# pymoc/pymoc

Measured on AMD Instinct MI355X. Metric: column-timesteps/sec (ensemble) at nz=100, higher is better.
Workload: dtype f64; 1 GPU; BASELINE configs[1]: 1024 independent Columns x nz=100 fp64 per GPU, static wA, do_conv on odd members, dt=30 d (pymoc_amd.configs.config2); columns_per_gpu=1024, nz=100, kernel=k_column_steps<64,2,6,true,true>, parallelism=ensemble sharded over 1 GPU(s), RCCL gather (root) of the final state

## Files before the change

### pymoc_amd/csrc/column.hip.h

```cpp
#pragma once
#include <type_traits>
#include "common.hip.h"

namespace pm {

template <int P>
struct ColGrid {
  double z[P];
  double dz[P];
  double dzc[P];
  double rdz[P], rdzc[P];
  double rdz_l[P], rdzc_l[P];
};
template <int P>
struct ColRegs {
  double b[P];
  double kap[P];
  double area[P];
  double dAk[P];
  double rarea[P];
  double rarea_l[P];
  double area_u, rarea_u, rarea_lu;
};

template <int P>
__device__ __forceinline__ void load_levels(double (&out)[P], const double *__restrict__ row,
                                            int lg, int nz, int lvl0 = 0) {
  if constexpr (P == 2) {
    if (lvl0 == 0 && (nz & 1) == 0 && (((unsigned long long)row) & 15ull) == 0ull) {
      const int i0 = lg * 2 < nz - 2 ? lg * 2 : nz - 2;
      const double2 v = *reinterpret_cast<const double2 *>(row + i0);
      out[0] = v.x;
      out[1] = v.y;
      return;
    }
  }
#pragma unroll
  for (int p = 0; p < P; ++p) {
    const int i = lvl0 + lg * P + p;
    out[p] = row[i < nz ? i : nz - 1];
  }
}

template <int P>
__device__ __forceinline__ double level_value(const double (&x)[P], int j) {
  const int jl = __builtin_amdgcn_readfirstlane(j / P);
  const int jp = __builtin_amdgcn_readfirstlane(j % P);
  double out = 0.;
#pragma unroll
  for (int p = 0; p < P; ++p) {
    const int lo = __builtin_amdgcn_readlane(__double2loint(x[p]), jl);
    const int hi = __builtin_amdgcn_readlane(__double2hiint(x[p]), jl);
    const double v = __hiloint2double(hi, lo);
    out = (p == 0 || jp == p) ? v : out;
  }
  return out;
}

__device__ __forceinline__ double lane_value(double x, int lane) {
  const int lo = __builtin_amdgcn_readlane(__double2loint(x), lane);
  const int hi = __builtin_amdgcn_readlane(__double2hiint(x), lane);
  return __hiloint2double(hi, lo);
}

template <int P>
struct ConvCache {
  unsigned long long mask[P];
  double zconv;
  bool valid = false;
};

template <int G, int P>
__device__ __forceinline__ bool col_convect(double (&b)[P], const double (&z)[P],
                                            double bs, double N2min, int lg, int lane,
                                            int nz, const double *__restrict__ zg,
                                            ConvCache<P> *cache = nullptr) {
  const unsigned long long gm = group_mask<G>(lane);
  bool ind[P];
  unsigned long long im[P];
  unsigned long long anym = 0ull;
#pragma unroll
  for (int p = 0; p < P; ++p) {
    const int i = lg * P + p;
    ind[p] = (i < nz) && (b[p] > bs);
    im[p] = __builtin_amdgcn_ballot_w64(ind[p]);
    anym |= im[p] & gm;
  }
  if (__builtin_expect(anym != 0ull, 0)) {
    double zconv;
    bool hit = false;
    if constexpr (G == 64) {
      if (cache != nullptr && cache->valid) {
        hit = true;
#pragma unroll
        for (int p = 0; p < P; ++p) hit = hit && (cache->mask[p] == im[p]);
      }
    }
    if (hit) {
      zconv = cache->zconv;
    } else {
      int jmax = 0;
#pragma unroll
      for (int p = 0; p < P; ++p) {
        const int i = lg * P + p;
        const unsigned long long m = __builtin_amdgcn_ballot_w64((i < nz) && !ind[p]) & gm;
        if (m != 0ull) {
          const int hl = 63 - __clzll((long long)m);
          const int j = (hl % G) * P + p;
          jmax = j > jmax ? j : jmax;
        }
      }
      if constexpr (G == 64) {
        zconv = level_value<P>(z, jmax);
        if (cache != nullptr) {
#pragma unroll
          for (int p = 0; p < P; ++p) cache->mask[p] = im[p];
          cache->zconv = zconv;
          cache->valid = true;
        }
      } else {
        zconv = zg[jmax];
      }
    }
#pragma unroll
    for (int p = 0; p < P; ++p) {
      const double adj = bs + N2min * (z[p] - zconv);
      b[p] = ind[p] ? adj : b[p];
    }
    return true;
  }
#pragma unroll
  for (int p = 0; p < P; ++p)
    if (lg * P + p == nz - 1) b[p] = bs;
  return false;
}

template <int P>
__device__ __forceinline__ void col_convect_cached(double (&b)[P], const double (&z)[P],
                                                   double bs, double N2min, int lane, int nz,
                                                   ConvCache<P> &cc) {
  bool ind[P];
  unsigned long long im[P], anym = 0ull;
  bool same = cc.valid;
#pragma unroll
  for (int p = 0; p < P; ++p) {
    ind[p] = (lane * P + p < nz) && (b[p] > bs);
    im[p] = __builtin_amdgcn_ballot_w64(ind[p]);
    anym |= im[p];
    same = same && (im[p] == cc.mask[p]);
  }
  if (__builtin_expect(!same, 0)) {
    int jmax = 0;
#pragma unroll
    for (int p = 0; p < P; ++p) {
      const unsigned long long m = __builtin_amdgcn_ballot_w64((lane * P + p < nz) && !ind[p]);
      if (m != 0ull) {
        const int j = (63 - __clzll((long long)m)) * P + p;
        jmax = j > jmax ? j : jmax;
      }
    }
    cc.zconv = level_value<P>(z, jmax);
#pragma unroll
    for (int p = 0; p < P; ++p) cc.mask[p] = im[p];
    cc.valid = true;
  }
  const bool none = anym == 0ull;
#pragma unroll
  for (int p = 0; p < P; ++p) {
    const double adj = bs + N2min * (z[p] - cc.zconv);
    b[p] = ind[p] ? adj : b[p];
    if (lane * P + p == nz - 1) b[p] = none ? bs : b[p];
  }
}

template <int G, int P, int DIV, bool BC = true, bool WEFF = false, bool UA = false,
          bool FLUXFMA = (DIV == 2 || DIV >= 6)>
__device__ __forceinline__ void col_vertadvdiff(const ColGrid<P> &g, ColRegs<P> &r,
                                                const double (&wA)[P],
                                                double dt, bool do_conv, double bs,
                                                double bbot, bool use_bzbot,
                                                double bzbot, int lg, int nz,
                                                int lvl0 = 0) {
  if (BC && !do_conv) {
#pragma unroll
    for (int p = 0; p < P; ++p)
      if (lvl0 + lg * P + p == nz - 1) r.b[p] = bs;
  }
  const double nb0 = from_next_lane_z(r.b[0]);
  double bup[P];
#pragma unroll
  for (int p = 0; p < P; ++p) bup[p] = (p < P - 1) ? r.b[p + 1 < P ? p + 1 : p] : nb0;
  if (BC && lvl0 + lg * P == 0) r.b[0] = use_bzbot ? (bup[0] - bzbot * g.dz[0]) : bbot;

  if constexpr (DIV == 4) {
    double d_up[P];
#pragma unroll
    for (int p = 0; p < P; ++p) d_up[p] = bup[p] - r.b[p];
    const double pd = from_prev_lane_z(d_up[P - 1]);
#pragma unroll
    for (int p = 0; p < P; ++p) {
      const double d_dn = (p > 0) ? d_up[p > 0 ? p - 1 : 0] : pd;
      r.b[p] = __builtin_fma(r.kap[p], d_up[p], __builtin_fma(r.dAk[p], d_dn, r.b[p]));
    }
    return;
  }
  double bz[P];
  {
    double num[P], q[P], rr[P];
#pragma unroll
    for (int p = 0; p < P; ++p) num[p] = bup[p] - r.b[p];
    if constexpr (DIV == 2) {
#pragma unroll
      for (int p = 0; p < P; ++p) rr[p] = num[p] * g.rdz_l[p];
#pragma unroll
      for (int p = 0; p < P; ++p) q[p] = __builtin_fma(num[p], g.rdz[p], rr[p]);
#pragma unroll
      for (int p = 0; p < P; ++p) rr[p] = __builtin_fma(-g.dz[p], q[p], num[p]);
#pragma unroll
      for (int p = 0; p < P; ++p) q[p] = __builtin_fma(rr[p], g.rdz[p], q[p]);
    } else if constexpr (DIV == 7 || DIV == 8) {
#pragma unroll
      for (int p = 0; p < P; ++p) rr[p] = num[p] * g.rdz_l[p];
#pragma unroll
      for (int p = 0; p < P; ++p) q[p] = __builtin_fma(num[p], g.rdz[p], rr[p]);
    } else if constexpr (DIV == 6) {
#pragma unroll
      for (int p = 0; p < P; ++p) q[p] = num[p] * g.rdz[p];
#pragma unroll
      for (int p = 0; p < P; ++p) rr[p] = __builtin_fma(-g.dz[p], q[p], num[p]);
#pragma unroll
      for (int p = 0; p < P; ++p) q[p] = __builtin_fma(rr[p], g.rdz[p], q[p]);
    } else if constexpr (DIV == 1 || DIV == 3 || DIV == 5) {
#pragma unroll
      for (int p = 0; p < P; ++p) q[p] = num[p] * g.rdz[p];
#pragma unroll
      for (int p = 0; p < P; ++p) rr[p] = __builtin_fma(-g.dz[p], q[p], num[p]);
#pragma unroll
      for (int p = 0; p < P; ++p) q[p] = __builtin_fma(rr[p], g.rdz[p], q[p]);
#pragma unroll
      for (int p = 0; p < P; ++p) rr[p] = __builtin_fma(-g.dz[p], q[p], num[p]);
#pragma unroll
      for (int p = 0; p < P; ++p) q[p] = __builtin_fma(rr[p], g.rdz[p], q[p]);
    } else {
#pragma unroll
      for (int p = 0; p < P; ++p) q[p] = num[p] / g.dz[p];
    }
    if constexpr (DIV != 0) {
#pragma unroll
      for (int p = 0; p < P; ++p) bz[p] = q[p];
    } else {
#pragma unroll
      for (int p = 0; p < P; ++p) bz[p] = (lvl0 + lg * P + p < nz - 1) ? q[p] : 0.0;
    }
  }
  const double pbz = from_prev_lane_z(bz[P - 1]);
  double bz_dn[P], dbz[P], flx[P], bzz[P], adv[P];
#pragma unroll
  for (int p = 0; p < P; ++p) {
    bz_dn[p] = (p > 0) ? bz[p > 0 ? p - 1 : 0] : pbz;
    dbz[p] = bz[p] - bz_dn[p];
    const double weff = WEFF ? wA[p] : wA[p] - r.dAk[p];
    if constexpr (FLUXFMA) {
      const double wn = (weff < 0.0) ? -weff : 0.0, wp = (weff < 0.0) ? 0.0 : -weff;
      flx[p] = __builtin_fma(wn, bz[p], wp * bz_dn[p]);
    } else {
      const double bzu = (weff < 0.0) ? bz[p] : bz_dn[p];
      flx[p] = (-weff) * bzu;
    }
  }
  if constexpr (DIV == 2) {
    double r1[P], r2[P];
#pragma unroll
    for (int p = 0; p < P; ++p) {
      r1[p] = dbz[p] * g.rdzc_l[p];
      r2[p] = flx[p] * (UA ? r.rarea_lu : r.rarea_l[p]);
    }
#pragma unroll
    for (int p = 0; p < P; ++p) {
      bzz[p] = __builtin_fma(dbz[p], g.rdzc[p], r1[p]);
      adv[p] = __builtin_fma(flx[p], (UA ? r.rarea_u : r.rarea[p]), r2[p]);
    }
#pragma unroll
    for (int p = 0; p < P; ++p) {
      r1[p] = __builtin_fma(-g.dzc[p], bzz[p], dbz[p]);
      r2[p] = __builtin_fma(-(UA ? r.area_u : r.area[p]), adv[p], flx[p]);
    }
#pragma unroll
    for (int p = 0; p < P; ++p) {
      bzz[p] = __builtin_fma(r1[p], g.rdzc[p], bzz[p]);
      adv[p] = __builtin_fma(r2[p], (UA ? r.rarea_u : r.rarea[p]), adv[p]);
    }
  } else if constexpr (DIV == 6) {
    double r1[P], r2[P];
#pragma unroll
    for (int p = 0; p < P; ++p) {
      bzz[p] = dbz[p] * g.rdzc[p];
      adv[p] = flx[p] * (UA ? r.rarea_u : r.rarea[p]);
    }
#pragma unroll
    for (int p = 0; p < P; ++p) {
      r1[p] = __builtin_fma(-g.dzc[p], bzz[p], dbz[p]);
      r2[p] = __builtin_fma(-(UA ? r.area_u : r.area[p]), adv[p], flx[p]);
    }
#pragma unroll
    for (int p = 0; p < P; ++p) {
      bzz[p] = __builtin_fma(r1[p], g.rdzc[p], bzz[p]);
      adv[p] = __builtin_fma(r2[p], (UA ? r.rarea_u : r.rarea[p]), adv[p]);
    }
  } else if constexpr (DIV == 8) {
    double r1[P], r2[P];
#pragma unroll
    for (int p = 0; p < P; ++p) {
      r1[p] = dbz[p] * g.rdzc_l[p];
      r2[p] = flx[p] * (UA ? r.rarea_lu : r.rarea_l[p]);
    }
#pragma unroll
    for (int p = 0; p < P; ++p) {
      bzz[p] = __builtin_fma(dbz[p], g.rdzc[p], r1[p]);
      adv[p] = __builtin_fma(flx[p], (UA ? r.rarea_u : r.rarea[p]), r2[p]);
    }
  } else if constexpr (DIV == 7) {
    double r1[P], r2[P];
#pragma unroll
    for (int p = 0; p < P; ++p) {
      r1[p] = dbz[p] * g.rdzc_l[p];
      adv[p] = flx[p] * (UA ? r.rarea_u : r.rarea[p]);
    }
#pragma unroll
    for (int p = 0; p < P; ++p) {
      bzz[p] = __builtin_fma(dbz[p], g.rdzc[p], r1[p]);
      r2[p] = __builtin_fma(-(UA ? r.area_u : r.area[p]), adv[p], flx[p]);
    }
#pragma unroll
    for (int p = 0; p < P; ++p) adv[p] = __builtin_fma(r2[p], (UA ? r.rarea_u : r.rarea[p]), adv[p]);
  } else if constexpr (DIV == 5) {
    double r1[P];
#pragma unroll
    for (int p = 0; p < P; ++p) {
      bzz[p] = dbz[p] * g.rdzc[p];
      adv[p] = div_by_recip2(flx[p], r.area_u, r.rarea_u, r.rarea_lu);
    }
#pragma unroll
    for (int k = 0; k < 2; ++k) {
#pragma unroll
      for (int p = 0; p < P; ++p) r1[p] = __builtin_fma(-g.dzc[p], bzz[p], dbz[p]);
#pragma unroll
      for (int p = 0; p < P; ++p) bzz[p] = __builtin_fma(r1[p], g.rdzc[p], bzz[p]);
    }
  } else if constexpr (DIV == 3) {
    double r1[P];
#pragma unroll
    for (int p = 0; p < P; ++p) {
      bzz[p] = dbz[p] * g.rdzc[p];
      adv[p] = flx[p] / (UA ? r.area_u : r.area[p]);
    }
#pragma unroll
    for (int k = 0; k < 2; ++k) {
#pragma unroll
      for (int p = 0; p < P; ++p) r1[p] = __builtin_fma(-g.dzc[p], bzz[p], dbz[p]);
#pragma unroll
      for (int p = 0; p < P; ++p) bzz[p] = __builtin_fma(r1[p], g.rdzc[p], bzz[p]);
    }
  } else if constexpr (DIV == 1) {
    double r1[P], r2[P];
#pragma unroll
    for (int p = 0; p < P; ++p) {
      bzz[p] = dbz[p] * g.rdzc[p];
      adv[p] = flx[p] * (UA ? r.rarea_u : r.rarea[p]);
    }
#pragma unroll
    for (int k = 0; k < 2; ++k) {
#pragma unroll
      for (int p = 0; p < P; ++p) {
        r1[p] = __builtin_fma(-g.dzc[p], bzz[p], dbz[p]);
        r2[p] = __builtin_fma(-(UA ? r.area_u : r.area[p]), adv[p], flx[p]);
      }
#pragma unroll
      for (int p = 0; p < P; ++p) {
        bzz[p] = __builtin_fma(r1[p], g.rdzc[p], bzz[p]);
        adv[p] = __builtin_fma(r2[p], (UA ? r.rarea_u : r.rarea[p]), adv[p]);
      }
    }
  } else {
#pragma unroll
    for (int p = 0; p < P; ++p) {
      bzz[p] = dbz[p] / g.dzc[p];
      adv[p] = flx[p] / (UA ? r.area_u : r.area[p]);
    }
  }
#pragma unroll
  for (int p = 0; p < P; ++p) {
    const int i = lvl0 + lg * P + p;
    const bool interior = (i >= 1) && (i <= nz - 2);
    const double db_dt = adv[p] + r.kap[p] * bzz[p];
    if constexpr (DIV == 0) {
      const double nb = r.b[p] + dt * db_dt;
      r.b[p] = interior ? nb : r.b[p];
    } else {
      r.b[p] = r.b[p] + (interior ? dt : 0.0) * db_dt;
    }
  }
}

template <int P>
__device__ __forceinline__ void col_horadv(ColRegs<P> &r, const double (&vdx)[P],
                                           const double (&bin)[P], double dt, int lg,
                                           int nz) {
#pragma unroll
  for (int p = 0; p < P; ++p) {
    const int i = lg * P + p;
    if (i < nz && vdx[p] > 0.0) {
      const double db = bin[p] - r.b[p];
      r.b[p] = r.b[p] + dt * vdx[p] * db / r.area[p];
    }
  }
}

template <int P>
__device__ __forceinline__ bool col_inputs_in_fast_range(const ColGrid<P> &g, const ColRegs<P> &r,
                                                         const double (&wA)[P], double dt,
                                                         double bs, double bbot, double bzbot,
                                                         double N2min, int lg, int nz) {
  bool ok = in_fast_div_range(dt) && in_fast_div_range(bs) && in_fast_div_range(bbot) &&
            in_fast_div_range(bzbot) && in_fast_div_range(N2min);
#pragma unroll
  for (int p = 0; p < P; ++p) {
    const bool top = lg * P + p >= nz - 1;
    ok = ok && in_fast_div_range(r.b[p]) && in_fast_div_range(wA[p]) &&
         in_fast_div_range(r.dAk[p]) && in_fast_div_range(wA[p] - r.dAk[p]) &&
         in_fast_div_range(r.kap[p]) && in_fast_div_range(r.area[p]) && r.area[p] != 0.0 &&
         in_fast_div_range(g.z[p]) && (top || (in_fast_div_range(g.dz[p]) && g.dz[p] != 0.0)) &&
         in_fast_div_range(g.dzc[p]) && g.dzc[p] != 0.0;
  }
  return ok;
}

template <int P>
__device__ __forceinline__ bool col_state_in_fast_range(const ColRegs<P> &r, const double (&wA)[P]) {
  int ok = 1;
#pragma unroll
  for (int p = 0; p < P; ++p)
    ok &= (int)in_fast_div_range(r.b[p]) & (int)in_fast_div_range(wA[p] - r.dAk[p]);
  return ok != 0;
}

template <int P, int DIV = 1>
__device__ __forceinline__ void col_load_grid(ColGrid<P> &g, const pm_columns &c, int lg,
                                              int lvl0 = 0) {
  const int nz = c.nz;
#pragma unroll
  for (int p = 0; p < P; ++p) {
    const int i = lvl0 + lg * P + p;
    const int ic = i < nz ? i : nz - 1;
    const int iu = ic + 1 < nz ? ic + 1 : nz - 1;
    const int id = ic > 0 ? ic - 1 : 0;
    const double zc = c.z[ic];
    g.z[p] = zc;
    g.dz[p] = c.z[iu] - zc;
    g.dzc[p] = 0.5 * (g.dz[p] + (zc - c.z[id]));
    if constexpr (DIV != 0 && DIV != 4) {
      g.rdz[p] = (i < nz - 1) ? 1.0 / g.dz[p] : 0.0;
      g.rdzc[p] = 1.0 / g.dzc[p];
    } else {
      g.rdz[p] = g.rdzc[p] = 0.0;
    }
    if constexpr (DIV == 2) {
      g.rdz_l[p] = (i < nz - 1) ? recip_lo(g.dz[p], g.rdz[p]) : 0.0;
      g.rdzc_l[p] = recip_lo(g.dzc[p], g.rdzc[p]);
    } else {
      g.rdz_l[p] = g.rdzc_l[p] = 0.0;
    }
  }
}

template <int P, int DIV = 1>
__device__ __forceinline__ void col_load_static(ColRegs<P> &r, const pm_columns &c,
                                                int col, int sel, int lg, int lvl0 = 0,
                                                bool uniform_area = false, bool weff_in = false) {
  const int nz = c.nz;
  const size_t base = (size_t)col * nz;
  const size_t sbase = ((size_t)sel * c.ncols + col) * nz;
  load_levels<P>(r.kap, c.kappa + sbase, lg, nz, lvl0);
  if (!weff_in) {
    load_levels<P>(r.dAk, c.dAkappa + sbase, lg, nz, lvl0);
  } else {
#pragma unroll
    for (int p = 0; p < P; ++p) r.dAk[p] = 0.0;
  }
  if (uniform_area) {
    const double a0 = c.area[base];
    const double ra = (DIV != 0 && DIV != 4) ? 1.0 / a0 : 0.0;
    const double ral = DIV == 2 ? recip_lo(a0, ra) : 0.0;
#pragma unroll
    for (int p = 0; p < P; ++p) {
      r.area[p] = a0;
      r.rarea[p] = ra;
      r.rarea_l[p] = ral;
    }
    return;
  }
  load_levels<P>(r.area, c.area + base, lg, nz, lvl0);
#pragma unroll
  for (int p = 0; p < P; ++p) {
    r.rarea[p] = (DIV != 0 && DIV != 4) ? 1.0 / r.area[p] : 0.0;
    r.rarea_l[p] = DIV == 2 ? recip_lo(r.area[p], r.rarea[p]) : 0.0;
  }
}

template <int P>
__device__ __forceinline__ void col_make_contracted(const ColGrid<P> &g, ColRegs<P> &r,
                                                    const double (&wA)[P], double dt, int lane,
                                                    int nz) {
  const double dz_prev_lane = from_prev_lane_z(g.dz[P - 1]);
#pragma unroll
  for (int p = 0; p < P; ++p) {
    const int i = lane * P + p;
    const bool interior = i >= 1 && i <= nz - 2;
    const double weff = wA[p] - r.dAk[p];
    const double dz_up = interior ? g.dz[p] : 1.0;
    const double dz_dn = interior ? ((p > 0) ? g.dz[p > 0 ? p - 1 : 0] : dz_prev_lane) : 1.0;
    const double dzc = interior ? g.dzc[p] : 1.0, area = interior ? r.area[p] : 1.0;
    const double wn = (weff < 0.0) ? -weff : 0.0, wp = (weff < 0.0) ? 0.0 : -weff;
    const double cu = dt * (r.kap[p] / (dzc * dz_up) + wn / (area * dz_up));
    const double cl = dt * (-r.kap[p] / (dzc * dz_dn) + wp / (area * dz_dn));
    r.kap[p] = interior ? cu : 0.0;
    r.dAk[p] = interior ? cl : 0.0;
  }
}

template <int P>
__device__ __forceinline__ unsigned conv_variant(const ConvCache<P> &cc) {
  unsigned need = 0u;
#pragma unroll
  for (int p = 0; p < P; ++p) need |= (cc.mask[p] != 0ull) ? (1u << p) : 0u;
  if constexpr (P <= 2) {
    return need;
  } else {
    return need ? (1u << P) - 1u : 0u;
  }
}

template <int P, int DIV, unsigned SEL, bool UA = false>
__device__ __forceinline__ int conv_spec_run(const ColGrid<P> &g, ColRegs<P> &r,
                                             const double (&wA)[P], double dt, double bs,
                                             double bbot, double N2min, int lane, int nz,
                                             ConvCache<P> &cc, int s, int nsteps) {
  constexpr int UNR = P <= 2 ? 16 : (P <= 4 ? 2 : 1);
  double adjv[P];
  double bs_eff[P];
  auto set_adj = [&]() {
#pragma unroll
    for (int p = 0; p < P; ++p)
      adjv[p] = (lane * P + p == 0) ? bbot : bs + N2min * (g.z[p] - cc.zconv);
  };
  set_adj();
#pragma unroll
  for (int p = 0; p < P; ++p) bs_eff[p] = (lane * P + p < nz) ? bs : __builtin_inf();
  double b_blk[P];
  unsigned long long acc;
  double bmax[P];
  auto spec = [&]() {
    unsigned long long im[P];
    bool ind[P];
#pragma unroll
    for (int p = 0; p < P; ++p) {
      if (((SEL >> p) & 1u) != 0u) {
        ind[p] = r.b[p] > bs_eff[p];
        im[p] = __builtin_amdgcn_ballot_w64(ind[p]);
      } else {
        bmax[p] = __builtin_fmax(bmax[p], r.b[p]);
      }
    }
#pragma unroll
    for (int p = 0; p < P; ++p) {
      if (((SEL >> p) & 1u) != 0u) r.b[p] = ind[p] ? adjv[p] : r.b[p];
    }
    col_vertadvdiff<64, P, DIV, false, false, UA>(g, r, wA, dt, true, bs, bbot, false, 0., lane, nz);
#pragma unroll
    for (int p = 0; p < P; ++p) {
      if (((SEL >> p) & 1u) != 0u) {
        unsigned long long x;
        asm("s_xor_b64 %0, %1, %2" : "=s"(x) : "s"(im[p]), "s"(cc.mask[p]) : "scc");
        acc |= x;
      }
    }
  };
  auto block_begin = [&]() {
    acc = 0ull;
#pragma unroll
    for (int p = 0; p < P; ++p) {
      b_blk[p] = r.b[p];
      bmax[p] = -__builtin_inf();
    }
  };
  auto block_bad = [&]() -> bool {
    bool conv = false;
#pragma unroll
    for (int p = 0; p < P; ++p)
      if (((SEL >> p) & 1u) == 0u) conv = conv || (bmax[p] > bs_eff[p]);
    if constexpr (SEL != (1u << P) - 1u) {
      unsigned long long any = __builtin_amdgcn_ballot_w64(conv);
      asm("" : "+s"(any));
      acc |= any;
    }
    return acc != 0ull;
  };
  auto redo = [&](int nb) {
#pragma unroll
    for (int p = 0; p < P; ++p) r.b[p] = b_blk[p];
    for (int k = 0; k < nb; ++k) {
      col_convect_cached<P>(r.b, g.z, bs, N2min, lane, nz, cc);
      if (lane == 0) r.b[0] = bbot;
      col_vertadvdiff<64, P, DIV, false, false, UA>(g, r, wA, dt, true, bs, bbot, false, 0., lane, nz);
    }
  };
  int pos = s, ret = -1;
  auto tier = [&](auto U) {
    constexpr int N = decltype(U)::value;
    int left = (nsteps - pos) / N;
    const int s_end = pos + left * N;
    for (; left > 0; --left) {
      block_begin();
#pragma unroll
      for (int k = 0; k < N; ++k) spec();
      if (__builtin_expect(block_bad(), 0)) {
        redo(N);
        if (conv_variant<P>(cc) != SEL) {
          ret = s_end - (left - 1) * N;
          left = 1;
        } else {
          set_adj();
        }
      }
    }
    pos = s_end;
  };
  if (UNR <= 4 || nsteps - pos >= 4 * UNR) tier(std::integral_constant<int, UNR>{});
  if (ret >= 0) return ret;
  if constexpr (UNR > 4) {
    tier(std::integral_constant<int, 4>{});
    if (ret >= 0) return ret;
  }
  if constexpr (UNR > 1) tier(std::integral_constant<int, 1>{});
  return ret >= 0 ? ret : nsteps;
}

template <int G, int P>
__device__ __forceinline__ void col_store_result(const pm_columns &c, const ColRegs<P> &r,
                                                 size_t base, int col, bool col_ok, int lg,
                                                 int lane, int nz) {
  bool bad = false;
  bool stored = false;
  if constexpr (P == 2) {
    if ((nz & 1) == 0 && (((unsigned long long)(c.b + base)) & 15ull) == 0ull) {
      if (lg * 2 < nz) {
        if (col_ok) *reinterpret_cast<double2 *>(c.b + base + lg * 2) = make_double2(r.b[0], r.b[1]);
        bad = !isfinite(r.b[0]) || !isfinite(r.b[1]);
      }
      stored = true;
    }
  }
  if (!stored) {
#pragma unroll
    for (int p = 0; p < P; ++p) {
      const int i = lg * P + p;
      if (i < nz) {
        if (col_ok) c.b[base + i] = r.b[p];
        bad |= !isfinite(r.b[p]);
      }
    }
  }
  if (c.nonfinite) {
    const unsigned long long m = __ballot(bad) & group_mask<G>(lane);
    if (lg == 0 && col_ok) c.nonfinite[col] = (m != 0ull) ? 1 : 0;
  }
}

template <int P>
__device__ __forceinline__ void col_pin(double (&b)[P]) {
#pragma unroll
  for (int p = 0; p < P; ++p) asm volatile("" : "+v"(b[p]));
}

template <int G, int P, int FAST, bool PLAIN, bool UA = false>
__global__ __launch_bounds__(256) void k_column_steps(
    pm_columns c, const double *__restrict__ wA_g, const double *__restrict__ vdx_g,
    const double *__restrict__ bin_g, double dt, int nsteps, int ops) {
  const int lane = threadIdx.x & (WAVE - 1);
  const int lg = threadIdx.x % G;
  int col_raw = (int)((blockIdx.x * (unsigned)blockDim.x + threadIdx.x) / G);
  constexpr bool FORMS = FAST == 6 && G == 64 && P <= 2 && PLAIN;
  if constexpr (FORMS) col_raw = __builtin_amdgcn_readfirstlane(col_raw);
  const bool col_ok = col_raw < c.ncols;
  const int col = col_ok ? col_raw : c.ncols - 1;
  const int nz = c.nz;
  const size_t base = (size_t)col * nz;

  ColGrid<P> g;
  ColRegs<P> r;
  const int sel = c.ksel ? c.ksel[col] : 0;
  const int flags = c.flags ? c.flags[col] : 0;
  col_load_grid<P, FAST>(g, c, lg);
  const bool ua = G == 64 && __builtin_amdgcn_readfirstlane(flags & PM_COL_UNIFORM_AREA) != 0;
  col_load_static<P, FAST>(r, c, col, sel, lg, 0, ua, (ops & PM_OP_WEFF) != 0);
  if constexpr (UA) {
    r.area_u = lane_value(r.area[0], 0);
    r.rarea_u = lane_value(r.rarea[0], 0);
    r.rarea_lu = lane_value(r.rarea_l[0], 0);
  }

  double wA[P], vdx[P], bin[P];
  load_levels<P>(r.b, c.b + base, lg, nz);
#pragma unroll
  for (int p = 0; p < P; ++p) wA[p] = vdx[p] = bin[p] = 0.0;
  const bool wA_row = !(PLAIN && (ops & PM_OP_WA_TWOBASIN) != 0 && col >= 2 * (c.ncols / 3));
  if (wA_g && wA_row) load_levels<P>(wA, wA_g + base, lg, nz);
  if constexpr (PLAIN) {
    if (ops & PM_OP_WA_PSI) {
      const int half = c.ncols >> 1;
      if (col < half) {
        if (bin_g) {
          double pso[P];
          load_levels<P>(pso, bin_g + base, lg, nz);
#pragma unroll
          for (int p = 0; p < P; ++p) wA[p] = (wA[p] - pso[p]) * 1e6;
        } else {
#pragma unroll
          for (int p = 0; p < P; ++p) wA[p] = wA[p] * 1e6;
        }
      } else {
#pragma unroll
        for (int p = 0; p < P; ++p) wA[p] = (-wA[p]) * 1e6;
      }
    }
  }
  if constexpr (PLAIN) {
    if (ops & PM_OP_WA_TWOBASIN) {
      const int third = c.ncols / 3;
      if (col < third) {
        double zon[P], pso[P];
        load_levels<P>(zon, vdx_g + base, lg, nz);
        load_levels<P>(pso, bin_g + base, lg, nz);
#pragma unroll
        for (int p = 0; p < P; ++p) wA[p] = (wA[p] + zon[p] - pso[p]) * 1e6;
      } else if (col < 2 * third) {
#pragma unroll
        for (int p = 0; p < P; ++p) wA[p] = (-wA[p]) * 1e6;
      } else {
        const size_t bp = (size_t)(col - third) * nz;
        double zon[P], pso[P];
        load_levels<P>(zon, vdx_g + bp, lg, nz);
        load_levels<P>(pso, bin_g + bp, lg, nz);
#pragma unroll
        for (int p = 0; p < P; ++p) wA[p] = (-zon[p] - pso[p]) * 1e6;
      }
    }
  }
  const bool wa_formed = (ops & (PM_OP_WA_PSI | PM_OP_WA_TWOBASIN)) != 0;
  if (vdx_g && !wa_formed) load_levels<P>(vdx, vdx_g + base, lg, nz);
  if (bin_g && !wa_formed) load_levels<P>(bin, bin_g + base, lg, nz);
  const bool do_conv = (flags & PM_COL_DO_CONV) != 0;
  const bool use_bzbot = (flags & PM_COL_BZBOT) != 0 && c.bzbot != nullptr;
  const double bs = c.bs[col];
  const double bbot = c.bbot[col];
  const double bzbot = use_bzbot ? c.bzbot[col] : 0.0;
  const double N2min = c.N2min[col];

  if constexpr (FAST != 0) {
    const bool vouched = G == 64 &&
                         __builtin_amdgcn_readfirstlane(flags & PM_COL_STATIC_IN_RANGE) != 0 &&
                         in_fast_div_range(dt);
    bool fast_ok;
    if (vouched)
      fast_ok = col_state_in_fast_range<P>(r, wA);
    else
      fast_ok = col_inputs_in_fast_range<P>(g, r, wA, dt, bs, bbot, bzbot, N2min, lg, nz);
    if (__builtin_expect(__ballot(!fast_ok) != 0ull, 0)) {
      for (int s = 0; s < nsteps; ++s) {
        if ((ops & PM_OP_CONVECT) && do_conv)
          col_convect<G, P>(r.b, g.z, bs, N2min, lg, lane, nz, c.z);
        col_pin<P>(r.b);
        if (ops & PM_OP_VERTADVDIFF)
          col_vertadvdiff<G, P, 0>(g, r, wA, dt, do_conv, bs, bbot, use_bzbot, bzbot, lg, nz);
        if ((ops & PM_OP_HORADV) && vdx_g) col_horadv<P>(r, vdx, bin, dt, lg, nz);
      }
      col_store_result<G, P>(c, r, base, col, col_ok, lg, lane, nz);
      return;
    }
  }

  if constexpr (FAST == 4) col_make_contracted<P>(g, r, wA, dt, lane, nz);

  auto plain_run = [&](auto DIVC) {
    constexpr int DIV = decltype(DIVC)::value;
    if (do_conv && use_bzbot) {
      for (int s = 0; s < nsteps; ++s) {
        col_convect<G, P>(r.b, g.z, bs, N2min, lg, lane, nz, c.z);
        col_vertadvdiff<G, P, DIV, true, false, UA>(g, r, wA, dt, true, bs, bbot, true, bzbot, lg, nz);
      }
    } else if (do_conv) {
      ConvCache<P> cc;
#pragma unroll
      for (int p = 0; p < P; ++p) cc.mask[p] = 0ull;
      cc.zconv = 0.;
      if constexpr (G == 64) {
        col_convect_cached<P>(r.b, g.z, bs, N2min, lane, nz, cc);
        if (lg == 0) r.b[0] = bbot;
        col_vertadvdiff<G, P, DIV, false, false, UA>(g, r, wA, dt, true, bs, bbot, false, 0., lg, nz);
        int s = 1;
        while (s < nsteps) {
          const unsigned v = conv_variant<P>(cc);
          if constexpr (P <= 2) {
            switch (v) {
              case 0: s = conv_spec_run<P, DIV, 0u, UA>(g, r, wA, dt, bs, bbot, N2min, lane, nz, cc, s, nsteps); break;
              case 1: s = conv_spec_run<P, DIV, 1u, UA>(g, r, wA, dt, bs, bbot, N2min, lane, nz, cc, s, nsteps); break;
              case 2: s = conv_spec_run<P, DIV, 2u, UA>(g, r, wA, dt, bs, bbot, N2min, lane, nz, cc, s, nsteps); break;
              default: s = conv_spec_run<P, DIV, 3u, UA>(g, r, wA, dt, bs, bbot, N2min, lane, nz, cc, s, nsteps); break;
            }
          } else {
            if (v == 0u)
              s = conv_spec_run<P, DIV, 0u, UA>(g, r, wA, dt, bs, bbot, N2min, lane, nz, cc, s, nsteps);
            else
              s = conv_spec_run<P, DIV, (1u << P) - 1u, UA>(g, r, wA, dt, bs, bbot, N2min, lane, nz, cc, s, nsteps);
          }
        }
      } else {
        for (int s = 0; s < nsteps; ++s) {
          col_convect<G, P>(r.b, g.z, bs, N2min, lg, lane, nz, c.z);
          if (lg == 0) r.b[0] = bbot;
          col_vertadvdiff<G, P, DIV, false, false, UA>(g, r, wA, dt, true, bs, bbot, false, 0., lg, nz);
        }
      }
    } else if (use_bzbot) {
      for (int s = 0; s < nsteps; ++s)
        col_vertadvdiff<G, P, DIV, true, false, UA>(g, r, wA, dt, false, bs, bbot, true, bzbot, lg, nz);
    } else {
#pragma unroll
      for (int p = 0; p < P; ++p) {
        if (lg * P + p == nz - 1) r.b[p] = bs;
        if (lg * P + p == 0) r.b[p] = bbot;
      }
      int s = 0;
      if constexpr (P <= 2) {
        for (; s + 4 <= nsteps; s += 4) {
          col_vertadvdiff<G, P, DIV, false, false, UA>(g, r, wA, dt, false, bs, bbot, false, 0., lg, nz);
          col_vertadvdiff<G, P, DIV, false, false, UA>(g, r, wA, dt, false, bs, bbot, false, 0., lg, nz);
          col_vertadvdiff<G, P, DIV, false, false, UA>(g, r, wA, dt, false, bs, bbot, false, 0., lg, nz);
          col_vertadvdiff<G, P, DIV, false, false, UA>(g, r, wA, dt, false, bs, bbot, false, 0., lg, nz);
        }
      }
      for (; s < nsteps; ++s)
        col_vertadvdiff<G, P, DIV, false, false, UA>(g, r, wA, dt, false, bs, bbot, false, 0., lg, nz);
    }
  };
  if constexpr (PLAIN) {
    if constexpr (FORMS) {
      const bool d2g = (c.reserved & PM_COLS_DIV3_PROVEN) != 0 && (c.reserved & PM_COLS_DIV2_GRID) != 0;
      if (d2g) {
#pragma unroll
        for (int p = 0; p < P; ++p) {
          const bool below_top = lg * P + p < nz - 1;
          g.rdz_l[p] = below_top ? recip_lo_div(g.dz[p], g.rdz[p]) : 0.0;
          g.rdzc_l[p] = below_top ? recip_lo_div(g.dzc[p], g.rdzc[p]) : 0.0;
        }
        if (__builtin_amdgcn_readfirstlane(flags & PM_COL_DIV2_AREA) != 0) {
          if constexpr (UA) {
            r.rarea_lu = lane_value(recip_lo_div(r.area_u, r.rarea_u), 0);
          } else {
#pragma unroll
            for (int p = 0; p < P; ++p) r.rarea_l[p] = recip_lo_div(r.area[p], r.rarea[p]);
          }
          plain_run(std::integral_constant<int, 8>{});
        } else {
          plain_run(std::integral_constant<int, 7>{});
        }
      } else {
        plain_run(std::integral_constant<int, 6>{});
      }
    } else {
      plain_run(std::integral_constant<int, FAST>{});
    }
  } else {
    for (int s = 0; s < nsteps; ++s) {
      if ((ops & PM_OP_CONVECT) && do_conv)
        col_convect<G, P>(r.b, g.z, bs, N2min, lg, lane, nz, c.z);
      col_pin<P>(r.b);
      if (ops & PM_OP_VERTADVDIFF)
        col_vertadvdiff<G, P, FAST, true, false, UA>(g, r, wA, dt, do_conv, bs, bbot, use_bzbot, bzbot, lg, nz);
      if ((ops & PM_OP_HORADV) && vdx_g) col_horadv<P>(r, vdx, bin, dt, lg, nz);
    }
  }

  col_store_result<G, P>(c, r, base, col, col_ok, lg, lane, nz);
}

template <int P>
struct ColStage {
  double b[P], wA[P], kap[P], area[P], dAk[P];
};
template <int P>
struct ColStageLean {
  double b[P], wA[P];
};

struct StreamScalars {
  int flags, sel;
  double bs, bbot, bzbot, N2min, area0, kbase;
  double ra, ral;
  __device__ __forceinline__ void load(const pm_columns &c, int col0, int cend, int lane) {
    const int col = col0 + lane < cend ? col0 + lane : cend - 1;
    flags = c.flags ? c.flags[col] : 0;
    sel = c.ksel ? c.ksel[col] : 0;
    bs = c.bs[col];
    bbot = c.bbot[col];
    N2min = c.N2min[col];
    bzbot = ((flags & PM_COL_BZBOT) != 0 && c.bzbot != nullptr) ? c.bzbot[col] : 0.0;
    area0 = (flags & PM_COL_UNIFORM_AREA) ? c.area[(size_t)col * c.nz] : 0.0;
    kbase = c.kappa_base ? c.kappa_base[col] : 0.0;
    ra = 1.0 / area0;
    ral = recip_lo(area0, ra);
  }
};

template <int P, bool AFF = false>
__device__ __forceinline__ void col_stage_load(ColStage<P> &s, const pm_columns &c,
                                               const double *__restrict__ wA_g, int col,
                                               int lane, bool weff_in, int flags, int sel,
                                               double area0) {
  const int nz = c.nz;
  const size_t base = (size_t)col * nz;
  const size_t sbase = ((size_t)sel * c.ncols + col) * nz;
  load_levels<P>(s.b, c.b + base, lane, nz);
  load_levels<P>(s.wA, wA_g + base, lane, nz);
  if constexpr (!AFF) load_levels<P>(s.kap, c.kappa + sbase, lane, nz);
  if ((flags & PM_COL_UNIFORM_AREA) == 0) {
    load_levels<P>(s.area, c.area + base, lane, nz);
  } else {
#pragma unroll
    for (int p = 0; p < P; ++p) s.area[p] = area0;
  }
  if (!weff_in) {
    load_levels<P>(s.dAk, c.dAkappa + sbase, lane, nz);
  } else {
#pragma unroll
    for (int p = 0; p < P; ++p) s.dAk[p] = 0.0;
  }
}

template <int P, int D, bool AFF = false, bool LEAN = false, bool VEC = false, bool D3 = false,
          int CPWU = 0, int WEFFT = -1, int UABT = -1>
__global__ __launch_bounds__(256) __attribute__((amdgpu_waves_per_eu((LEAN && P <= 2 && D <= 5) ? 4 : 1)))
void k_column_stream(pm_columns c,
                                                       const double *__restrict__ wA_g,
                                                       double dt, int nsteps, int cpw, bool dt_ok,
                                                       bool weff_in) {
  const int lane = threadIdx.x & (WAVE - 1);
  const int wave = (int)((blockIdx.x * (unsigned)blockDim.x + threadIdx.x) >> 6);
  const int col0 = __builtin_amdgcn_readfirstlane(wave * cpw);
  const int nz = c.nz;
  if (col0 >= c.ncols) return;
  const int cend = col0 + cpw < c.ncols ? col0 + cpw : c.ncols;

  StreamScalars sc;
  sc.load(c, col0, cend, lane);
  static_assert(!LEAN || AFF, "the lean ring needs the affine kappa");
  static_assert(!VEC || (LEAN && P == 2), "16-byte accesses: the lean form with two levels per lane");
  const int off2 = lane * 2 < nz - 2 ? lane * 2 : nz - 2;
  using Stage = typename std::conditional<LEAN, ColStageLean<P>, ColStage<P>>::type;
  auto flags_of = [&](int k) { return __builtin_amdgcn_readlane(sc.flags, k); };
  auto issue = [&](Stage &st, int col) {
    const int k = col - col0;
    if constexpr (VEC) {
      const size_t base = (size_t)col * nz;
      const double2 vb = *reinterpret_cast<const double2 *>(c.b + base + off2);
      const double2 vw = *reinterpret_cast<const double2 *>(wA_g + base + off2);
      st.b[0] = vb.x;
      st.b[P - 1] = vb.y;
      st.wA[0] = vw.x;
      st.wA[P - 1] = vw.y;
    } else if constexpr (LEAN) {
      const size_t base = (size_t)col * nz;
      load_levels<P>(st.b, c.b + base, lane, nz);
      load_levels<P>(st.wA, wA_g + base, lane, nz);
    } else if constexpr (CPWU > 0 && WEFFT >= 0 && UABT >= 0) {
      const int sel = __builtin_amdgcn_readlane(sc.sel, k);
      const size_t base = (size_t)col * nz, sbase = ((size_t)sel * c.ncols + col) * nz;
      load_levels<P>(st.b, c.b + base, lane, nz);
      load_levels<P>(st.wA, wA_g + base, lane, nz);
      if constexpr (!AFF) load_levels<P>(st.kap, c.kappa + sbase, lane, nz);
      if constexpr (UABT == 0) load_levels<P>(st.area, c.area + base, lane, nz);
      if constexpr (WEFFT == 0) load_levels<P>(st.dAk, c.dAkappa + sbase, lane, nz);
    } else {
      col_stage_load<P, AFF>(st, c, wA_g, col, lane, weff_in, flags_of(k),
                             __builtin_amdgcn_readlane(sc.sel, k), lane_value(sc.area0, k));
    }
  };
  ColGrid<P> g;
  col_load_grid<P, 1>(g, c, lane);
  double kprof[P];
#pragma unroll
  for (int p = 0; p < P; ++p) kprof[p] = 0.0;
  if constexpr (AFF) load_levels<P>(kprof, c.kappa_profile, lane, nz);
  Stage ring[D];
#pragma unroll
  for (int d = 0; d < D; ++d)
    if (col0 + d < cend) issue(ring[d], col0 + d);
  unsigned nf_bits = 0u;
  auto one_column = [&](int col, int d, bool prefetch, int kk) {
      ColRegs<P> r;
      double wA[P];
#pragma unroll
      for (int p = 0; p < P; ++p) {
        r.b[p] = ring[d].b[p];
        wA[p] = ring[d].wA[p];
        if constexpr (AFF)
          r.kap[p] = lane_value(sc.kbase, col - col0) + kprof[p];
        else
          r.kap[p] = ring[d].kap[p];
        if constexpr (LEAN) {
          r.area[p] = lane_value(sc.area0, col - col0);
          r.area_u = r.area[p];
          r.rarea_u = lane_value(sc.ra, col - col0);
          r.rarea_lu = lane_value(sc.ral, col - col0);
          r.dAk[p] = 0.0;
        } else if constexpr (CPWU > 0 && WEFFT >= 0 && UABT >= 0) {
          if constexpr (UABT == 1)
            r.area[p] = lane_value(sc.area0, col - col0);
          else
            r.area[p] = ring[d].area[p];
          if constexpr (WEFFT == 1)
            r.dAk[p] = 0.0;
          else
            r.dAk[p] = ring[d].dAk[p];
        } else {
          r.area[p] = ring[d].area[p];
          r.dAk[p] = ring[d].dAk[p];
        }
        r.rarea[p] = r.rarea_l[p] = 0.;
      }
      if (CPWU > 0) {
        if (prefetch) issue(ring[d], col + D);
      } else {
        issue(ring[d], col + D < cend ? col + D : cend - 1);
      }
      const int k = col - col0;
      const int flags = flags_of(k);
      const bool do_conv = (flags & PM_COL_DO_CONV) != 0;
      const bool use_bzbot = (flags & PM_COL_BZBOT) != 0 && c.bzbot != nullptr;
      const double bs = lane_value(sc.bs, k), bbot = lane_value(sc.bbot, k),
                   N2min = lane_value(sc.N2min, k), bzbot = lane_value(sc.bzbot, k);
      const bool fast_ok = ((flags & PM_COL_STATIC_IN_RANGE) != 0 && dt_ok)
                               ? col_state_in_fast_range<P>(r, wA)
                               : col_inputs_in_fast_range<P>(g, r, wA, dt, bs, bbot, bzbot, N2min,
                                                             lane, nz);
      const bool slow = __ballot(!fast_ok) != 0ull;
      for (int s = 0; s < nsteps; ++s) {
        if (do_conv) col_convect<64, P>(r.b, g.z, bs, N2min, lane, lane, nz, c.z);
        col_pin<P>(r.b);
        if (__builtin_expect(slow, 0))
          col_vertadvdiff<64, P, 0>(g, r, wA, dt, do_conv, bs, bbot, use_bzbot, bzbot, lane, nz);
        else if constexpr (LEAN && D3)
          col_vertadvdiff<64, P, 6, true, false, true, false>(g, r, wA, dt, do_conv, bs, bbot, use_bzbot,
                                                              bzbot, lane, nz);
        else if constexpr (LEAN)
          col_vertadvdiff<64, P, 5, true, false, true>(g, r, wA, dt, do_conv, bs, bbot, use_bzbot,
                                                       bzbot, lane, nz);
        else
          col_vertadvdiff<64, P, 3>(g, r, wA, dt, do_conv, bs, bbot, use_bzbot, bzbot, lane, nz);
      }
      const size_t base = (size_t)col * nz;
      bool bad = false;
      bool stored = false;
      if constexpr (VEC) {
        if (lane * 2 < nz) {
          *reinterpret_cast<double2 *>(c.b + base + lane * 2) = make_double2(r.b[0], r.b[P - 1]);
          bad = !isfinite(r.b[0]) || !isfinite(r.b[P - 1]);
        }
        stored = true;
      } else if constexpr (P == 2) {
        if ((nz & 1) == 0 && (((unsigned long long)(c.b + base)) & 15ull) == 0ull) {
          if (lane * 2 < nz) {
            *reinterpret_cast<double2 *>(c.b + base + lane * 2) = make_double2(r.b[0], r.b[1]);
            bad = !isfinite(r.b[0]) || !isfinite(r.b[1]);
          }
          stored = true;
        }
      }
      if (!stored) {
#pragma unroll
        for (int p = 0; p < P; ++p) {
          const int i = lane * P + p;
          if (i < nz) {
            c.b[base + i] = r.b[p];
            bad |= !isfinite(r.b[p]);
          }
        }
      }
      if (CPWU > 0) {
        nf_bits |= (__ballot(bad) != 0ull ? 1u : 0u) << kk;
      } else if (c.nonfinite) {
        const unsigned long long m = __ballot(bad);
        if (lane == 0) c.nonfinite[col] = (m != 0ull) ? 1 : 0;
      }
  };
  if constexpr (CPWU > 0) {
#pragma unroll
    for (int k = 0; k < CPWU; ++k) one_column(col0 + k, k % D, k + D < CPWU, k);
    if (c.nonfinite && lane < CPWU) c.nonfinite[col0 + lane] = (int)((nf_bits >> lane) & 1u);
  } else {
    for (int colb = col0; colb < cend; colb += D) {
#pragma unroll
      for (int d = 0; d < D; ++d) {
        const int col = colb + d;
        if (col >= cend) break;
        one_column(col, d, true, 0);
      }
    }
  }
}

inline int stream_cols_per_wave(int ncols) {
  const int waves_wanted = 1024 * 8;
  int cpw = ncols / waves_wanted;
  return cpw < 1 ? 1 : (cpw > 32 ? 32 : cpw);
}

inline int pick_levels_per_lane(int G, int need) {
  static const int sup64[] = {1, 2, 3, 4, 5, 6, 7, 8, 10, 13, 16};
  static const int sup[] = {1, 2, 3, 4, 5, 6, 7, 8};
  if (G == 64) {
    for (int v : sup64)
      if (v >= need) return v;
  } else {
    for (int v : sup)
      if (v >= need) return v;
  }
  return -1;
}

struct ColKernel {
  bool stream, plain, ua, aff, lean, vec, d3;
  int fast, d, cpwu, wefft, uabt;
  constexpr bool compiled(int G, int P) const {
    if (!stream && !ua && fast <= 2) return true;
    return G == 64 && P <= 4 && (P == 2 || (!vec && cpwu == 0));
  }
};
constexpr ColKernel col_steps(int fast, bool plain, bool ua = false) {
  return {false, plain, ua, false, false, false, false, fast, 0, 0, -1, -1};
}
constexpr ColKernel col_stream(int d, bool aff = false, bool lean = false, bool vec = false,
                               bool d3 = false, int cpwu = 0, int wefft = -1, int uabt = -1) {
  return {true, false, false, aff, lean, vec, d3, 0, d, cpwu, wefft, uabt};
}

#define PM_COLUMN_KERNELS(X)                                                                   \
  X(CK_STEPS_IEEE, col_steps(0, false))                                         \
  X(CK_STEPS_RECIP, col_steps(1, false))              \
  X(CK_STEPS_PLAIN, col_steps(2, true))                              \
  X(CK_STEPS_PLAIN_UA, col_steps(2, true, true))                \
  X(CK_STEPS_DIV3_UA, col_steps(6, true, true))           \
  X(CK_STEPS_CONTRACTED, col_steps(4, true))                         \
  X(CK_STREAM, col_stream(2))                                \
  X(CK_STREAM_WEFF, col_stream(3))                                    \
  X(CK_STREAM_AFF, col_stream(3, true))                 \
  X(CK_STREAM_WEFF_AFF, col_stream(4, true))                                                   \
  X(CK_STREAM_LEAN, col_stream(5, true, true))            \
  X(CK_STREAM_LEAN_VEC, col_stream(5, true, true, true))             \
  X(CK_STREAM_LEAN_VEC_D3, col_stream(5, true, true, true, true))                              \
  X(CK_STREAM_LEAN_VEC_U8, col_stream(5, true, true, true, false, 8))       \
  X(CK_STREAM_LEAN_VEC_D3_U8, col_stream(5, true, true, true, true, 8))                        \
  X(CK_STREAM_U8, col_stream(2, false, false, false, false, 8, 0, 0))                          \
  X(CK_STREAM_WEFF_UA_U8, col_stream(3, false, false, false, false, 8, 1, 1))

#define PM_CK_ID(id, args) id,
enum ColKernelId { CK_NONE, PM_COLUMN_KERNELS(PM_CK_ID) };
#undef PM_CK_ID
constexpr ColKernel col_kernel(ColKernelId k) {
#define PM_CK_ARGS(id, args) \
  case id: return args;
  switch (k) {
    PM_COLUMN_KERNELS(PM_CK_ARGS)
    default: return {};
  }
#undef PM_CK_ARGS
}

struct ColumnPlan {
  ColKernelId kernel;
  int G, P;
  int cpw;
  unsigned grid;
};

inline ColumnPlan column_plan(const pm_columns &c, const double *wA, const double *vdx, int nsteps,
                              int ops, int G, int P) {
  const bool weff = (ops & PM_OP_WEFF) != 0;
  const bool plain =
      (ops & ~(PM_OP_WEFF | PM_OP_CONTRACTED | PM_OP_WA_PSI | PM_OP_WA_TWOBASIN)) == PM_OP_TIMESTEP &&
      (!vdx || (ops & PM_OP_WA_TWOBASIN));
  const bool ua = (c.reserved & PM_COLS_ALL_UNIFORM_AREA) != 0;
  const bool d3 = (c.reserved & PM_COLS_DIV3_PROVEN) != 0;
  const bool aff = c.kappa_base && c.kappa_profile && c.nsel == 1;
  const bool wave_per_col = G == 64 && P <= 4;
  const int cpw = stream_cols_per_wave(c.ncols);
  ColumnPlan pl{CK_STEPS_IEEE, G, P, 0, (unsigned)((c.ncols + 256 / G - 1) / (256 / G))};
  if (wave_per_col && nsteps < 3 && plain && cpw >= 2) {
    pl.cpw = cpw;
    if (weff && aff && ua) {
      pl.cpw = c.ncols / 16384 < 2 ? 2 : (c.ncols / 16384 > 16 ? 16 : c.ncols / 16384);
      const bool vec = P == 2 && (c.nz & 1) == 0 &&
                       ((((unsigned long long)c.b) | ((unsigned long long)wA)) & 15ull) == 0ull;
      const bool u8 = vec && c.ncols % 8 == 0 && c.ncols >= 8 * 4096;
      if (u8) pl.cpw = 8;
      pl.kernel = !vec ? CK_STREAM_LEAN
                  : u8 ? (d3 ? CK_STREAM_LEAN_VEC_D3_U8 : CK_STREAM_LEAN_VEC_U8)
                       : (d3 ? CK_STREAM_LEAN_VEC_D3 : CK_STREAM_LEAN_VEC);
    } else if (P == 2 && !aff && c.ncols % 8 == 0 && c.ncols >= 8 * 4096 && weff == ua) {
      pl.cpw = 8;
      pl.kernel = weff ? CK_STREAM_WEFF_UA_U8 : CK_STREAM_U8;
    } else {
      pl.kernel = weff ? (aff ? CK_STREAM_WEFF_AFF : CK_STREAM_WEFF) : (aff ? CK_STREAM_AFF : CK_STREAM);
    }
    const unsigned waves = (unsigned)((c.ncols + pl.cpw - 1) / pl.cpw);
    pl.grid = (waves + 3) / 4;
  } else if (nsteps >= 3 && plain) {
    if (wave_per_col && (ops & PM_OP_CONTRACTED))
      pl.kernel = CK_STEPS_CONTRACTED;
    else if (wave_per_col && ua)
      pl.kernel = d3 ? CK_STEPS_DIV3_UA : CK_STEPS_PLAIN_UA;
    else
      pl.kernel = CK_STEPS_PLAIN;
  } else if (nsteps >= 3) {
    pl.kernel = CK_STEPS_RECIP;
  }
  return pl;
}

inline int column_kernel_name(const ColumnPlan &pl, char *name, size_t len) {
  const ColKernel k = col_kernel(pl.kernel);
  auto tf = [](bool v) { return v ? "true" : "false"; };
  int n = 0;
  if (pl.kernel == CK_NONE)
    n = snprintf(name, len, "%s", "");
  else if (k.stream)
    n = snprintf(name, len, "k_column_stream<%d,%d,%s,%s,%s,%s,%d,%d,%d>", pl.P, k.d, tf(k.aff),
                 tf(k.lean), tf(k.vec), tf(k.d3), k.cpwu, k.wefft, k.uabt);
  else
    n = snprintf(name, len, "k_column_steps<%d,%d,%d,%s,%s>", pl.G, pl.P, k.fast, tf(k.plain),
                 tf(k.ua));
  PM_REQUIRE(n >= 0 && (size_t)n < len, "name buffer of %zu bytes too small", len);
  return PM_OK;
}

template <int G, int P, ColKernelId K>
int launch_column_kernel(const ColumnPlan &pl, const pm_columns &c, const double *wA,
                         const double *vdx, const double *bin, double dt, int nsteps, int ops,
                         hipStream_t st) {
  constexpr ColKernel k = col_kernel(K);
  if constexpr (!k.compiled(G, P)) {
    return fail(PM_EINVAL, "column kernel %d is not compiled for G=%d P=%d", (int)K, G, P);
  } else if constexpr (k.stream) {
    const double adt = dt < 0 ? -dt : dt;
    const bool dt_ok = dt == 0.0 || (adt >= 0x1p-200 && adt <= 0x1p200);
    hipLaunchKernelGGL((k_column_stream<P, k.d, k.aff, k.lean, k.vec, k.d3, k.cpwu, k.wefft, k.uabt>),
                       dim3(pl.grid), dim3(256), 0, st, c, wA, dt, nsteps, pl.cpw, dt_ok,
                       (ops & PM_OP_WEFF) != 0);
  } else {
    hipLaunchKernelGGL((k_column_steps<G, P, k.fast, k.plain, k.ua>), dim3(pl.grid), dim3(256), 0,
                       st, c, wA, vdx, bin, dt, nsteps, ops & ~PM_OP_CONTRACTED);
  }
  PM_HIP(hipGetLastError());
  return PM_OK;
}

template <int G, int P>
int launch_column_steps(const ColumnPlan &pl, const pm_columns &c, const double *wA,
                        const double *vdx, const double *bin, double dt, int nsteps, int ops,
                        hipStream_t st) {
#define PM_CK_LAUNCH(id, args) \
  case id: return launch_column_kernel<G, P, id>(pl, c, wA, vdx, bin, dt, nsteps, ops, st);
  switch (pl.kernel) {
    PM_COLUMN_KERNELS(PM_CK_LAUNCH)
    default: return PM_OK;
  }
#undef PM_CK_LAUNCH
}

int column_steps_g16(const ColumnPlan &pl, const pm_columns &c, const double *wA,
                     const double *vdx, const double *bin, double dt, int nsteps, int ops,
                     hipStream_t st);
int column_steps_g32(const ColumnPlan &pl, const pm_columns &c, const double *wA,
                     const double *vdx, const double *bin, double dt, int nsteps, int ops,
                     hipStream_t st);
int column_steps_g64(const ColumnPlan &pl, const pm_columns &c, const double *wA,
                     const double *vdx, const double *bin, double dt, int nsteps, int ops,
                     hipStream_t st);

}
```

Baseline: 13.88 billion column-timesteps/s.

## Run no-convection fast path when only the surface cell stays convectively held

Adds detection of the steady case where the only convecting cell is the top one, pinned at the surface value. In that case the speculative run uses the cheaper SEL=0 variant and excludes the top level from the instability test, instead of running the masked convection variant. This avoids per-step ballots and adjustments in columns that sit at a persistent surface convective state. If the held state breaks, the block redoes and falls back; correctness depends on the cached zconv and mask semantics matching the excluded cell. The extra ballot in the dispatch loop adds a small cost.

```diff
diff --git a/pymoc_amd/csrc/column.hip.h b/pymoc_amd/csrc/column.hip.h
--- a/pymoc_amd/csrc/column.hip.h
+++ b/pymoc_amd/csrc/column.hip.h
@@ -529,12 +529,40 @@
 }
 
 template <int P>
-__device__ __forceinline__ unsigned conv_variant(const ConvCache<P> &cc) {
+__device__ __forceinline__ bool conv_surface_only(const ConvCache<P> &cc, int nz) {
+  if constexpr (P > 2) {
+    return false;
+  } else {
+    const int top = nz - 1;
+    bool only = cc.valid && top > 0;
+#pragma unroll
+    for (int p = 0; p < P; ++p)
+      only = only && (cc.mask[p] == ((top % P == p) ? (1ull << (top / P)) : 0ull));
+    return only;
+  }
+}
+template <int P>
+__device__ __forceinline__ bool conv_held(const ConvCache<P> &cc, const double (&b)[P], double bs,
+                                          int nz) {
+  if constexpr (P > 2) {
+    return false;
+  } else {
+    const int top = nz - 1;
+    unsigned long long above = 0ull;
+#pragma unroll
+    for (int p = 0; p < P; ++p)
+      above |= (top % P == p) ? (__builtin_amdgcn_ballot_w64(b[p] > bs) >> (top / P)) & 1ull : 0ull;
+    return above != 0ull && conv_surface_only<P>(cc, nz);
+  }
+}
+
+template <int P>
+__device__ __forceinline__ unsigned conv_variant(const ConvCache<P> &cc, bool held) {
   unsigned need = 0u;
 #pragma unroll
   for (int p = 0; p < P; ++p) need |= (cc.mask[p] != 0ull) ? (1u << p) : 0u;
   if constexpr (P <= 2) {
-    return need;
+    return held ? 0u : need;
   } else {
     return need ? (1u << P) - 1u : 0u;
   }
@@ -544,7 +572,7 @@
 __device__ __forceinline__ int conv_spec_run(const ColGrid<P> &g, ColRegs<P> &r,
                                              const double (&wA)[P], double dt, double bs,
                                              double bbot, double N2min, int lane, int nz,
-                                             ConvCache<P> &cc, int s, int nsteps) {
+                                             ConvCache<P> &cc, int s, int nsteps, bool held) {
   constexpr int UNR = P <= 2 ? 16 : (P <= 4 ? 2 : 1);
   double adjv[P];
   double bs_eff[P];
@@ -554,8 +582,9 @@
       adjv[p] = (lane * P + p == 0) ? bbot : bs + N2min * (g.z[p] - cc.zconv);
   };
   set_adj();
-#pragma unroll
-  for (int p = 0; p < P; ++p) bs_eff[p] = (lane * P + p < nz) ? bs : __builtin_inf();
+  const int nz_test = nz - ((SEL == 0u && held) ? 1 : 0);
+#pragma unroll
+  for (int p = 0; p < P; ++p) bs_eff[p] = (lane * P + p < nz_test) ? bs : __builtin_inf();
   double b_blk[P];
   unsigned long long acc;
   double bmax[P];
@@ -625,11 +654,15 @@
       for (int k = 0; k < N; ++k) spec();
       if (__builtin_expect(block_bad(), 0)) {
         redo(N);
-        if (conv_variant<P>(cc) != SEL) {
+        if (conv_variant<P>(cc, false) != SEL || conv_surface_only<P>(cc, nz)) {
           ret = s_end - (left - 1) * N;
           left = 1;
         } else {
           set_adj();
+          if constexpr (SEL == 0u && P <= 2) {
+#pragma unroll
+            for (int p = 0; p < P; ++p) bs_eff[p] = (lane * P + p < nz) ? bs : __builtin_inf();
+          }
         }
       }
     }
@@ -809,19 +842,20 @@
         col_vertadvdiff<G, P, DIV, false, false, UA>(g, r, wA, dt, true, bs, bbot, false, 0., lg, nz);
         int s = 1;
         while (s < nsteps) {
-          const unsigned v = conv_variant<P>(cc);
+          const bool held = conv_held<P>(cc, r.b, bs, nz);
+          const unsigned v = conv_variant<P>(cc, held);
           if constexpr (P <= 2) {
             switch (v) {
-              case 0: s = conv_spec_run<P, DIV, 0u, UA>(g, r, wA, dt, bs, bbot, N2min, lane, nz, cc, s, nsteps); break;
-              case 1: s = conv_spec_run<P, DIV, 1u, UA>(g, r, wA, dt, bs, bbot, N2min, lane, nz, cc, s, nsteps); break;
-              case 2: s = conv_spec_run<P, DIV, 2u, UA>(g, r, wA, dt, bs, bbot, N2min, lane, nz, cc, s, nsteps); break;
-              default: s = conv_spec_run<P, DIV, 3u, UA>(g, r, wA, dt, bs, bbot, N2min, lane, nz, cc, s, nsteps); break;
+              case 0: s = conv_spec_run<P, DIV, 0u, UA>(g, r, wA, dt, bs, bbot, N2min, lane, nz, cc, s, nsteps, held); break;
+              case 1: s = conv_spec_run<P, DIV, 1u, UA>(g, r, wA, dt, bs, bbot, N2min, lane, nz, cc, s, nsteps, held); break;
+              case 2: s = conv_spec_run<P, DIV, 2u, UA>(g, r, wA, dt, bs, bbot, N2min, lane, nz, cc, s, nsteps, held); break;
+              default: s = conv_spec_run<P, DIV, 3u, UA>(g, r, wA, dt, bs, bbot, N2min, lane, nz, cc, s, nsteps, held); break;
             }
           } else {
             if (v == 0u)
-              s = conv_spec_run<P, DIV, 0u, UA>(g, r, wA, dt, bs, bbot, N2min, lane, nz, cc, s, nsteps);
+              s = conv_spec_run<P, DIV, 0u, UA>(g, r, wA, dt, bs, bbot, N2min, lane, nz, cc, s, nsteps, held);
             else
-              s = conv_spec_run<P, DIV, (1u << P) - 1u, UA>(g, r, wA, dt, bs, bbot, N2min, lane, nz, cc, s, nsteps);
+              s = conv_spec_run<P, DIV, (1u << P) - 1u, UA>(g, r, wA, dt, bs, bbot, N2min, lane, nz, cc, s, nsteps, held);
           }
         }
       } else {
```

After: 13.92 billion column-timesteps/s, median of 6. Within noise of the previous version (+0.3%).
